# avi2924/Speech-Intent-Recognizer

Measured on AMD Instinct MI355X. Metric: utterances/sec (16 kHz, 3 s clips), inference: HIP STFT+mel+CNN/BiGRU forward + argmax, higher is better.
Workload: dtype f32

## Files before the change

speech-intent-recognizer_amd/csrc/api.hip:

```cpp
#include "sir_internal.h"
#include "model_shape.h"

#include <math.h>
#include <stdarg.h>
#include <stdio.h>
#include <string.h>
#include <algorithm>
#include <vector>

static thread_local char g_err[512] = "";

void sir_set_error(const char* fmt, ...) {
    va_list ap;
    va_start(ap, fmt);
    vsnprintf(g_err, sizeof(g_err), fmt, ap);
    va_end(ap);
}

int sir_check_hip(hipError_t e, const char* what) {
    if (e == hipSuccess) return SIR_OK;
    sir_set_error("HIP error %d (%s) at %s", (int)e, hipGetErrorString(e), what);
    return SIR_EHIP;
}

extern "C" int sir_abi_version(void) { return SIR_ABI_VERSION; }
extern "C" const char* sir_last_error(void) { return g_err; }

template <typename T>
static int upload(T** dst, const std::vector<T>& src) {
    SIR_HIP_TRY(hipMalloc((void**)dst, src.size() * sizeof(T)));
    SIR_HIP_TRY(hipMemcpy(*dst, src.data(), src.size() * sizeof(T), hipMemcpyHostToDevice));
    return SIR_OK;
}

bool sir_conv_stage_fits(int conv, bool shape_ok) {
    static const int forced = getenv("SIR_CONV_FALLBACK") ? atoi(getenv("SIR_CONV_FALLBACK")) : 0;
    return shape_ok && forced < (conv == 2 ? 1 : 2);
}

extern "C" int sir_create(const sir_feature_config* cfg, sir_handle** out) { return sir_create_ex(cfg, 0, out); }

extern "C" int sir_create_ex(const sir_feature_config* cfg, int win_length, sir_handle** out) {
    if (!cfg || !out) { sir_set_error("sir_create: NULL argument"); return SIR_EINVAL; }
    const int n_fft = cfg->n_fft, hop = cfg->hop_length;
    if (win_length == 0) win_length = n_fft;
    if ((n_fft != 256 && n_fft != 512 && n_fft != 1024) || hop < n_fft / 16 || hop > n_fft || win_length < 1 || win_length > n_fft) {
        sir_set_error("sir_create: n_fft=%d hop_length=%d win_length=%d is not built; supported: n_fft in {256, 512, 1024}, "
                      "n_fft/16 <= hop_length <= n_fft, 1 <= win_length <= n_fft", n_fft, hop, win_length);
        return SIR_EUNSUPPORTED;
    }
    if (cfg->n_mels < 1 || cfg->n_mels > SIR_MAX_MELS || cfg->sample_rate <= 0) {
        sir_set_error("sir_create: n_mels=%d sample_rate=%d out of range", cfg->n_mels, cfg->sample_rate);
        return SIR_EINVAL;
    }
    const int nfreq = n_fft / 2 + 1;
    sir_handle* h = new sir_handle();
    h->prof_mode = 0; h->prof_only = -1;
    h->weights_version = 0; h->prep_next = 0;
    for (auto& e : h->prep) { e.ws = nullptr; e.version = 0; e.key = -1; }
    h->tw512 = nullptr; h->tw1024 = nullptr; h->window = nullptr; h->melw = nullptr; h->mel_desc = nullptr;
    h->mel_taps = nullptr; h->mel_max_cover = 0;
    h->win_length = win_length;
    h->general = !(n_fft == SIR_NFFT && hop == SIR_HOP && win_length == SIR_NFFT);
    h->gen_twn = nullptr; h->gen_tw2n = nullptr;
    h->status = nullptr;
    h->cluster_done = nullptr; h->cluster_stream = nullptr; h->cluster_pending = false;
    h->cluster_seen = false; h->cluster_multi = false; h->cluster_run = 0;
    h->zero_page = nullptr; h->num_cus = 256;
    for (auto& x : h->xbufs) { x.st = nullptr; x.p = nullptr; x.kind = 0; x.cap = 0; x.bytes = 0; x.epoch = 0; x.used = 0; }
    h->xbuf_clock = 0;
    h->xbuf_evictions = 0;
    h->bwd_side = nullptr;
    for (auto& e : h->bwd_ev) e = nullptr;
    h->cfg = *cfg;
    h->cfg.window = nullptr;
    h->cfg.mel_fb = nullptr;
    if (sir_check_hip(hipGetDevice(&h->device), "hipGetDevice") != SIR_OK) { delete h; return SIR_EHIP; }

    const double PI = 3.14159265358979323846;
    std::vector<float2> tw512(512), tw1024(SIR_NFREQ);
    for (int j = 0; j < 512; ++j) tw512[j] = make_float2((float)cos(-2.0 * PI * j / 512.0), (float)sin(-2.0 * PI * j / 512.0));
    for (int k = 0; k < SIR_NFREQ; ++k) tw1024[k] = make_float2((float)cos(-2.0 * PI * k / 1024.0), (float)sin(-2.0 * PI * k / 1024.0));
    std::vector<float> window(n_fft, 0.0f);
    const int wleft = (n_fft - win_length) / 2;
    for (int n = 0; n < win_length; ++n)
        window[wleft + n] = cfg->window ? cfg->window[n] : (float)(0.5 - 0.5 * cos(2.0 * PI * n / win_length));
    std::vector<float2> gen_twn, gen_tw2n;
    if (h->general) {
        const int np = n_fft / 2;
        gen_twn.resize(np); gen_tw2n.resize(np);
        for (int k = 0; k < np; ++k) {
            gen_twn[k] = make_float2((float)cos(-2.0 * PI * k / np), (float)sin(-2.0 * PI * k / np));
            gen_tw2n[k] = make_float2((float)cos(-2.0 * PI * k / n_fft), (float)sin(-2.0 * PI * k / n_fft));
        }
    }

    const int nm = cfg->n_mels;
    std::vector<float> fb((size_t)nfreq * nm);
    if (cfg->mel_fb) {
        memcpy(fb.data(), cfg->mel_fb, fb.size() * sizeof(float));
    } else {
        const double f_lo = cfg->f_min, f_hi = cfg->f_max > 0 ? cfg->f_max : cfg->sample_rate / 2;
        const double mmin = 2595.0 * log10(1.0 + f_lo / 700.0), mmax = 2595.0 * log10(1.0 + f_hi / 700.0);
        std::vector<double> fpts(nm + 2);
        for (int i = 0; i < nm + 2; ++i) fpts[i] = 700.0 * (pow(10.0, (mmin + (mmax - mmin) * i / (nm + 1)) / 2595.0) - 1.0);
        for (int k = 0; k < nfreq; ++k) {
            const double f = (double)(cfg->sample_rate / 2) * k / (nfreq - 1);
            for (int j = 0; j < nm; ++j) {
                const double up = (f - fpts[j]) / (fpts[j + 1] - fpts[j]), down = (fpts[j + 2] - f) / (fpts[j + 2] - fpts[j + 1]);
                const double v = up < down ? up : down;
                fb[(size_t)k * nm + j] = (float)(v > 0.0 ? v : 0.0);
            }
        }
    }
    std::vector<int> start(SIR_MAX_MELS, 0), count(SIR_MAX_MELS, 0);
    for (int j = 0; j < nm; ++j) {
        int lo = -1, hi = -1;
        for (int k = 0; k < nfreq; ++k)
            if (fb[(size_t)k * nm + j] != 0.0f) { if (lo < 0) lo = k; hi = k; }
        if (lo >= 0) { start[j] = lo; count[j] = hi - lo + 1; }
    }
    std::vector<int> order(SIR_MAX_MELS);
    for (int j = 0; j < SIR_MAX_MELS; ++j) order[j] = j;
    std::stable_sort(order.begin(), order.end(), [&](int a, int b) {
        const int ca = a < nm ? count[a] : -1, cb = b < nm ? count[b] : -1;
        return ca < cb;
    });
    std::vector<float> melw;
    std::vector<int4> desc(SIR_MAX_MELS);
    for (int s = 0; s < SIR_MAX_MELS; ++s) {
        const int j = order[s];
        if (j >= nm) { desc[s] = make_int4(-1, 0, 0, 0); continue; }
        desc[s] = make_int4(j, start[j], count[j], (int)melw.size());
        for (int i = 0; i < count[j]; ++i) melw.push_back(fb[(size_t)(start[j] + i) * nm + j]);
    }
    if (melw.size() > 4096) {
        sir_set_error("sir_create: the mel filterbank has %zu taps; only banded (triangular) banks of <= 4096 taps are built", melw.size());
        delete h;
        return SIR_EUNSUPPORTED;
    }
    h->mel_nnz = (int)melw.size();
    if (h->general && sir_features_gen_lds_bytes(n_fft, h->mel_nnz) > SIR_LDS_BYTES) {
// ... 246 lines not shown
```

speech-intent-recognizer_amd/csrc/gru_quad.hip:

```cpp
#include <stdlib.h>
#include "gru_quad_kernel.h"
#include "gru_bwd_quad_kernel.h"

int sir_launch_gru_quad(sir_handle* h, hipStream_t st, bool save, const float* gi, const float* whh0, const float* whh1, const float* bhh0,
                        const float* bhh1, float* y, int B, int S, float* gates, unsigned short* yplanes, const void* wfrag0,
                        const void* wfrag1, const int* nlive, bool ragged) {
    if (ragged && (save || !nlive)) { sir_set_error("gru_quad: the ragged form is inference only and needs the step counts"); return SIR_EINVAL; }
    if (S >= 511) { sir_set_error("gru_quad: %d steps exceed the 9-bit step field of the granule tag", S); return SIR_EUNSUPPORTED; }
    if (!wfrag0 || !wfrag1) { sir_set_error("gru_quad: the prepared W_hh fragments are required (sir_prep_whh_quad / train_prep_kernel)"); return SIR_EINVAL; }
    const int clusters = ((B + GQ_NU - 1) / GQ_NU) * 2;
    const dim3 grid(4 * (unsigned)clusters);
    static const int dbg0 = getenv("SIR_GRU_DBG") ? atoi(getenv("SIR_GRU_DBG")) : 0;
    const int dbg = (dbg0 & ~(31 << 8)) | ((((dbg0 >> 8) & 31) ? ((dbg0 >> 8) & 31) : GQ_POLL_DELAY) << 8);
    typedef void (*kern_t)(const float*, const float*, const float*, const float*, const float*, float*, int, int, float*, unsigned long long*,
                           unsigned int*, int, unsigned, unsigned short*, const uint4*, const uint4*, const int*);
    const kern_t kern = save ? gru_quad_kernel<true, true> : ragged ? gru_quad_kernel<false, false, true> : gru_quad_kernel<false, false>;
    SIR_TRY(sir_lds_opt_in(h, (const void*)kern, (int)GQ_LDS_BYTES));
    SIR_TRY(sir_cluster_enter(h, st));
    unsigned epoch = 0;
    void* xbuf = nullptr;
    int rc = sir_xbuf_acquire(h, st, 1, (size_t)clusters * GQ_XBUF_PER_CLUSTER, 127u, &xbuf, &epoch);
    if (rc == SIR_OK) {
        hipLaunchKernelGGL(kern, grid, dim3(GQ_THREADS), GQ_LDS_BYTES, st, gi, whh0, whh1, bhh0, bhh1, y, B, S, gates,
                           (unsigned long long*)xbuf, h->status, dbg, epoch, yplanes, (const uint4*)wfrag0, (const uint4*)wfrag1, nlive);
        rc = sir_check_hip(hipGetLastError(), "gru_quad_kernel");
    }
    const int rc_leave = sir_cluster_leave(h, st);
    return rc != SIR_OK ? rc : rc_leave;
}

void sir_prep_whh_quad(hipStream_t st, const float* whh, void* frag) {
    hipLaunchKernelGGL(prep_whh_quad_kernel, dim3(GQ_FRAG_THREADS / 256), dim3(256), 0, st, whh, (uint4*)frag);
}

int sir_launch_gru_bwd_quad(sir_handle* h, hipStream_t st, const float* dy, const float* gates, const float* y, const float* whh0,
                            const float* whh1, float* dgi, float* dgh, float* bsum_i, float* bsum_h, int B, int S, const void* wfrag0,
                            const void* wfrag1) {
    if (S >= 65535) { sir_set_error("gru_bwd_quad: %d steps exceed the 16-bit step field of the granule tag", S); return SIR_EUNSUPPORTED; }
    if (!wfrag0 || !wfrag1) { sir_set_error("gru_bwd_quad: the prepared W_hh fragments are required (train_prep_kernel)"); return SIR_EINVAL; }
    const int clusters = ((B + GQ_NU - 1) / GQ_NU) * 2;
    const int dbg = GQ_POLL_DELAY << 8;
    SIR_TRY(sir_lds_opt_in(h, (const void*)gru_bwd_quad_kernel, (int)BQ_LDS_BYTES));
    SIR_TRY(sir_cluster_enter(h, st));
    unsigned epoch = 0;
    void* xbuf = nullptr;
    int rc = sir_xbuf_acquire(h, st, 3, (size_t)clusters * BQ_XBUF_PER_CLUSTER, 0xFFFFu, &xbuf, &epoch);
    if (rc == SIR_OK) {
        hipLaunchKernelGGL(gru_bwd_quad_kernel, dim3(4 * (unsigned)clusters), dim3(GQ_THREADS), BQ_LDS_BYTES, st, dy, gates, y, whh0, whh1, dgi, dgh,
                           bsum_i, bsum_h, B, S, (unsigned long long*)xbuf, h->status, epoch, dbg, (const uint4*)wfrag0, (const uint4*)wfrag1);
        rc = sir_check_hip(hipGetLastError(), "gru_bwd_quad_kernel");
    }
    const int rc_leave = sir_cluster_leave(h, st);
    return rc != SIR_OK ? rc : rc_leave;
}
```

speech-intent-recognizer_amd/csrc/gru_quad_kernel.h:

```cpp
#pragma once
#include "bf16x6_kernels.h"
#include "gru_frag_prep.h"

typedef unsigned int gq_u32x4 __attribute__((ext_vector_type(4)));
constexpr int GQ_NU = 16;
constexpr int GQ_UQ = 64;
constexpr int GQ_THREADS = 256;
constexpr int GQ_ROWB = 256 * 2 + 32;
constexpr int GQ_PLANEB = GQ_NU * GQ_ROWB;
constexpr int GQ_NPL = 2;
constexpr int GQ_BUFB = GQ_NPL * GQ_PLANEB;
constexpr size_t GQ_LDS_PLANES = 2 * (size_t)GQ_BUFB;
constexpr int GQ_TROW = 64 + 4;
constexpr size_t GQ_LDS_BYTES = GQ_LDS_PLANES + (size_t)GQ_NU * 3 * GQ_TROW * 4;
constexpr unsigned GQ_SPIN_LIMIT = 1u << 22;
constexpr int GQ_POLL_DELAY = 8;
constexpr size_t GQ_XBUF_PER_CLUSTER = (size_t)2 * 4 * GQ_NU * GQ_UQ * 8;

typedef float f32x4_t __attribute__((ext_vector_type(4)));

__device__ __forceinline__ void gq_mfma_aw(f32x4_t& acc, const f16x8& w, const f16x8& h) {
    asm volatile("v_mfma_f32_16x16x32_f16 %0, %1, %2, %0" : "+v"(acc) : "a"(w), "v"(h));
}
__device__ __forceinline__ void gq_mfma_wa(f32x4_t& acc, const f16x8& h, const f16x8& w) {
    asm volatile("v_mfma_f32_16x16x32_f16 %0, %1, %2, %0" : "+v"(acc) : "v"(h), "a"(w));
}
__device__ __forceinline__ void gq_mfma_enter(f32x4_t (&a)[3], f32x4_t (&b)[3]) {
    asm volatile("s_nop 3" : "+v"(a[0]), "+v"(a[1]), "+v"(a[2]), "+v"(b[0]), "+v"(b[1]), "+v"(b[2]));
}
__device__ __forceinline__ void gq_mfma_fence(f32x4_t (&a)[3], f32x4_t (&b)[3]) {
    asm volatile("s_nop 15" : "+v"(a[0]), "+v"(a[1]), "+v"(a[2]), "+v"(b[0]), "+v"(b[1]), "+v"(b[2]));
}
__device__ __forceinline__ void gq_mfma_enter(f32x4_t (&a)[4], f32x4_t (&b)[4]) {
    asm volatile("s_nop 3" : "+v"(a[0]), "+v"(a[1]), "+v"(a[2]), "+v"(a[3]), "+v"(b[0]), "+v"(b[1]), "+v"(b[2]), "+v"(b[3]));
}
__device__ __forceinline__ void gq_mfma_fence(f32x4_t (&a)[4], f32x4_t (&b)[4]) {
    asm volatile("s_nop 15" : "+v"(a[0]), "+v"(a[1]), "+v"(a[2]), "+v"(a[3]), "+v"(b[0]), "+v"(b[1]), "+v"(b[2]), "+v"(b[3]));
}

__device__ __forceinline__ float gq_sigmoid(float x) {
    return __builtin_amdgcn_rcpf(1.0f + __builtin_amdgcn_exp2f(-1.44269504088896341f * x));
}
__device__ __forceinline__ float gq_tanh(float x) {
    return 1.0f - 2.0f * __builtin_amdgcn_rcpf(1.0f + __builtin_amdgcn_exp2f(2.88539008177792681f * x));
}

static __global__ __launch_bounds__(256) void prep_whh_quad_kernel(const float* __restrict__ whh, uint4* __restrict__ frag) {
    prep_whh_quad_elem(whh, frag, blockIdx.x * 256 + threadIdx.x);
}

template <bool SAVE, bool ROLES = false, bool RAGGED = false>
__global__ __launch_bounds__(GQ_THREADS) void gru_quad_kernel(
    const float* __restrict__ gi, const float* __restrict__ whh0, const float* __restrict__ whh1,
    const float* __restrict__ bhh0, const float* __restrict__ bhh1, float* __restrict__ y, int B, int S,
    float* __restrict__ gates, unsigned long long* xbuf, unsigned int* status, int dbg, unsigned epoch, unsigned short* __restrict__ yplanes,
    const uint4* __restrict__ wfrag0, const uint4* __restrict__ wfrag1, const int* __restrict__ nlive) {
    extern __shared__ __attribute__((aligned(16))) unsigned char qlds[];
    const int nclusters = gridDim.x >> 2;
    const bool xcd_order = (nclusters & 7) == 0 && !(dbg & 32);
    const int q = xcd_order ? (blockIdx.x >> 3) & 3 : blockIdx.x & 3;
    const int cluster = xcd_order ? (blockIdx.x & 7) + 8 * (blockIdx.x >> 5) : blockIdx.x >> 2;
    const int dir = cluster & 1, grp = cluster >> 1;
    const int tid = threadIdx.x, lane = tid & 63, wv = tid >> 6;
    const int n = lane & 15, kg = lane >> 4;
    const int gutt = ROLES ? 4 * wv + (lane >> 4) : n;
    const int gul0 = ROLES ? 4 * (lane & 15) : wv * 16 + kg * 4;
    const int b = grp * GQ_NU + gutt;
    const bool bvalid = b < B;
    const int u0 = q * GQ_UQ + gul0;
    float* const tl = reinterpret_cast<float*>(qlds + GQ_LDS_PLANES);
    const float* __restrict__ bhh = dir ? bhh1 : bhh0;
    unsigned long long* xc = xbuf + (size_t)cluster * (2 * 4 * GQ_NU * GQ_UQ);

    int sr_ = S;
    if constexpr (RAGGED) {
        const int ui = grp * GQ_NU + (lane & 15);
        sr_ = ui < B ? min(S, nlive[ui]) : 0;
#pragma unroll
        for (int o = 8; o > 0; o >>= 1) sr_ = max(sr_, __shfl_xor(sr_, o));
        sr_ = max(sr_, min(S, 2));
    }
    const int SR = sr_;

    f16x8 wf[3][8][GQ_NPL];
    {
        const uint4* wsrc = (dir ? wfrag1 : wfrag0) + (size_t)((q * 4 + wv) * 3 * 8 * GQ_NPL) * 64 + lane;
#pragma unroll
        for (int g = 0; g < 3; ++g)
#pragma unroll
            for (int s = 0; s < 8; ++s)
#pragma unroll
                for (int p = 0; p < GQ_NPL; ++p)
                    asm volatile("global_load_dwordx4 %0, %1, off" : "=a"(wf[g][s][p]) : "v"(wsrc + ((g * 8 + s) * GQ_NPL + p) * 64));
        asm volatile("s_waitcnt vmcnt(0)" ::: "memory");
    }
    float4 bh[3];
#pragma unroll
    for (int g = 0; g < 3; ++g) bh[g] = *reinterpret_cast<const float4*>(bhh + g * 256 + u0);
    for (int i = tid; i < (int)(GQ_LDS_BYTES / 16); i += GQ_THREADS) reinterpret_cast<uint4*>(qlds)[i] = make_uint4(0, 0, 0, 0);
    float4 hprev = make_float4(0.f, 0.f, 0.f, 0.f);
    __syncthreads();

    float4 gin[3];
    const int nlb = (!SAVE && nlive && bvalid) ? nlive[b] : (RAGGED ? 0 : S);
    auto load_gi = [&](int t, float4 (&dst)[3]) {
#pragma unroll
        for (int g = 0; g < 3; ++g) dst[g] = make_float4(0.f, 0.f, 0.f, 0.f);
        if (RAGGED ? (bvalid && t < nlb) : bvalid) {
            const float* gp = gi + ((size_t)(RAGGED || t < nlb ? b : B) * S + t) * 1536 + dir * 768 + u0;
#pragma unroll
            for (int g = 0; g < 3; ++g) dst[g] = *reinterpret_cast<const float4*>(gp + g * 256);
        }
    };
    load_gi(dir ? SR - 1 : 0, gin);
    const int frag_off = n * GQ_ROWB + kg * 16;
    const int xoff = wv * 256 + lane * 2;
    bool timed_out = false;

    for (int step = 0; step < SR; ++step) {
        const int t = dir ? (SR - 1 - step) : step;
        float4 gcur[3] = {gin[0], gin[1], gin[2]};
        const unsigned char* hb = qlds + (step & 1) * GQ_BUFB;
        unsigned char* hnb = qlds + ((step + 1) & 1) * GQ_BUFB;

        f32x4_t acc[3], accx[3];
#pragma unroll
        for (int g = 0; g < 3; ++g) { acc[g] = (f32x4_t){0.f, 0.f, 0.f, 0.f}; accx[g] = (f32x4_t){0.f, 0.f, 0.f, 0.f}; }
        f16x8 hf[8][GQ_NPL];
        if (!(dbg & 2)) {
#pragma unroll
        for (int s = 0; s < 8; ++s)
#pragma unroll
            for (int p = 0; p < GQ_NPL; ++p)
                hf[s][p] = __builtin_bit_cast(f16x8, *reinterpret_cast<const uint4*>(hb + p * GQ_PLANEB + frag_off + s * 64));
        __builtin_amdgcn_sched_barrier(0);
        gq_mfma_enter(acc, accx);
#pragma unroll
        for (int s = 0; s < 8; ++s) {
#pragma unroll
            for (int g = 0; g < 3; ++g) gq_mfma_aw(accx[g], wf[g][s][1], hf[s][0]);
#pragma unroll
            for (int g = 0; g < 3; ++g) gq_mfma_aw(accx[g], wf[g][s][0], hf[s][1]);
#pragma unroll
            for (int g = 0; g < 3; ++g) gq_mfma_aw(acc[g], wf[g][s][0], hf[s][0]);
        }
        gq_mfma_fence(acc, accx);
#pragma unroll
        for (int g = 0; g < 3; ++g)
#pragma unroll
            for (int j = 0; j < 4; ++j) acc[g][j] = fmaf(accx[g][j], H3_LO_INV, acc[g][j]);
        }
        if constexpr (ROLES) {
#pragma unroll
            for (int g = 0; g < 3; ++g)
                *reinterpret_cast<float4*>(tl + (n * 3 + g) * GQ_TROW + wv * 16 + kg * 4) = make_float4(acc[g][0], acc[g][1], acc[g][2], acc[g][3]);
            __syncthreads();
#pragma unroll
            for (int g = 0; g < 3; ++g) {
                const float4 v = *reinterpret_cast<const float4*>(tl + (gutt * 3 + g) * GQ_TROW + gul0);
                acc[g][0] = v.x; acc[g][1] = v.y; acc[g][2] = v.z; acc[g][3] = v.w;
            }
        }

        float hn4[4], r4[4], z4[4], n4[4], hh4[4];
        const float gr[4] = {gcur[0].x, gcur[0].y, gcur[0].z, gcur[0].w}, gz[4] = {gcur[1].x, gcur[1].y, gcur[1].z, gcur[1].w};
        const float gn[4] = {gcur[2].x, gcur[2].y, gcur[2].z, gcur[2].w};
        const float br[4] = {bh[0].x, bh[0].y, bh[0].z, bh[0].w}, bz[4] = {bh[1].x, bh[1].y, bh[1].z, bh[1].w};
        const float bn[4] = {bh[2].x, bh[2].y, bh[2].z, bh[2].w};
        const float hp[4] = {hprev.x, hprev.y, hprev.z, hprev.w};
#pragma unroll
        for (int j = 0; j < 4; ++j) {
            const float hr = acc[0][j] + br[j], hz = acc[1][j] + bz[j];
            hh4[j] = acc[2][j] + bn[j];
            r4[j] = gq_sigmoid(gr[j] + hr);
            z4[j] = gq_sigmoid(gz[j] + hz);
            n4[j] = gq_tanh(gn[j] + r4[j] * hh4[j]);
            hn4[j] = (1.0f - z4[j]) * n4[j] + z4[j] * hp[j];
            if (RAGGED) hn4[j] = t < nlb ? hn4[j] : hp[j];
        }
        hprev = make_float4(hn4[0], hn4[1], hn4[2], hn4[3]);

        uint2 ph, pl;
        split2h_quad(hprev, ph, pl);
        {
// ... 92 lines not shown
```

speech-intent-recognizer_amd/csrc/model_infer.hip:

```cpp
#include "f16x3_kernels.h"
#include "conv_fwd.h"
#include "gru_frag_prep.h"

namespace {

enum WsBuf {
    WS_A1 = 0,
    WS_A2,
    WS_X0,
    WS_GI,
    WS_Y0,
    WS_Y1,
    WS_CTX,
    WS_PAD,
    WS_XZ,
    WS_BN,
    WS_WHT,
    WS_XS,
    WS_WS,
    WS_WCB,
    WS_GXB,
    WS_GFL,
    WS_COUNT
};

struct Dims : SirDims {
    int tw2, tw3, k2max, k3max;
};

bool make_dims(int batch, int t_frames, Dims* d) {
    if (!sir_make_dims(batch, t_frames, d)) return false;
    d->tw2 = (d->wp1 + 1) / 2; d->tw3 = (d->wp2 + 1) / 2; d->k2max = (d->tw2 + 3) / 4; d->k3max = (d->tw3 + 3) / 4;
    return true;
}

struct PadTabs { size_t e0, d1, d3, tab2, tab3, rows, count; };
PadTabs pad_tabs(const Dims& d) {
    PadTabs t;
    const size_t n = (size_t)d.B + 1;
    t.e0 = 0; t.d1 = d.B; t.d3 = t.d1 + n; t.rows = t.d3 + n + 1 + n * d.k2max + 1 + n * d.k3max;
    t.tab2 = t.rows + 1 + n * d.S; t.tab2 += t.tab2 & 1;
    t.tab3 = t.tab2 + 2 + 2 * n * d.k2max;
    t.count = t.tab3 + 2 + 2 * n * d.k3max;
    return t;
}

void ws_sizes(const Dims& d, size_t* bytes) {
    const size_t B = d.B + 1;
    bytes[WS_A1] = B * 32 * d.wp1 * 32 * 4;
    bytes[WS_A2] = B * 16 * d.wp2 * 64 * 4;
    bytes[WS_X0] = B * d.S * 1024 * 4;
    bytes[WS_GI] = B * d.S * 1536 * 4;
    bytes[WS_Y0] = (size_t)d.B * d.S * 512 * 4;
    bytes[WS_Y1] = (size_t)d.B * d.S * 512 * 4;
    bytes[WS_CTX] = (size_t)d.B * 512 * 4;
    bytes[WS_PAD] = pad_tabs(d).count * 4;
    bytes[WS_XZ] = (size_t)64 * d.T * 4;
    bytes[WS_BN] = (size_t)2 * 224 * 4;
    bytes[WS_WHT] = 4 * GRU_FRAG_BYTES;
    bytes[WS_XS] = B * d.S * 1024 * 2 * 2;
    bytes[WS_WS] = ((size_t)2 * 2 * 768 * 1024 + (size_t)2 * 2 * 768 * 512) * 2;
    bytes[WS_WCB] = ((size_t)3 * 32 * 16 * 64 + (size_t)3 * 64 * 16 * 128 + (size_t)3 * 64 * 9 * 128) * 2;
    bytes[WS_GXB] = 0;
    bytes[WS_GFL] = 0;
}

size_t ws_layout(const Dims& d, size_t* off) {
    size_t bytes[WS_COUNT], pos = 0;
    ws_sizes(d, bytes);
    for (int i = 0; i < WS_COUNT; ++i) {
        off[i] = pos;
        pos += sir_align_up(bytes[i], 256);
    }
    return pos;
}

static __global__ __launch_bounds__(256) void pad_extent_kernel(const float* __restrict__ x, int T, int* __restrict__ e0) {
    const unsigned* xb = reinterpret_cast<const unsigned*>(x) + (size_t)blockIdx.x * 64 * T;
    int last = -1;
    for (int c = threadIdx.x; c < T; c += 256) {
        unsigned acc = 0;
#pragma unroll 32
        for (int r = 0; r < 64; ++r) acc |= xb[(size_t)r * T + c];
        if (acc) last = c;
    }
#pragma unroll
    for (int o = 32; o > 0; o >>= 1) last = max(last, __shfl_xor(last, o));
    __shared__ int wl[4];
    if ((threadIdx.x & 63) == 0) wl[threadIdx.x >> 6] = last;
    __syncthreads();
    if (threadIdx.x == 0) e0[blockIdx.x] = max(max(wl[0], wl[1]), max(wl[2], wl[3])) + 1;
}

__device__ __forceinline__ int pk_cap(int r) { const int l = r & 3; return l == 1 ? 2 : l == 2 ? 1 : 0; }
__device__ __forceinline__ int pk_take(int c, int g, int cn) { return g <= c ? min(pk_cap(c - g), cn) : 0; }
constexpr int PK_ID = 0 | 1 << 2 | 2 << 4;
__device__ __forceinline__ int pk_fn(int c, int cn) { return pk_take(c, 0, cn) | pk_take(c, 1, cn) << 2 | pk_take(c, 2, cn) << 4; }
__device__ __forceinline__ int pk_then(int f, int g) {
    int r = 0;
#pragma unroll
    for (int x = 0; x < 3; ++x) r |= ((g >> (2 * ((f >> (2 * x)) & 3))) & 3) << (2 * x);
    return r;
}
__device__ __forceinline__ void pk_emit(int* __restrict__ tab, int o, int base, int g, int r, int gB, int nB) {
    const int k = (r + 3) >> 2;
    for (int t = 0; t < k; ++t) {
        reinterpret_cast<int2*>(tab)[1 + o + t] = make_int2((base + g + 4 * t) << 2 | (min(4, r - 4 * t) - 1),
                                                            t == k - 1 && nB > 0 ? gB << 2 | (2 - nB) << 1 | (nB - 1) : -1);
    }
}

template <bool PACK, typename Need>
__device__ __forceinline__ void pad_tables_emit(const Dims& d, int nu, Need need, int* __restrict__ d1o, int* __restrict__ d3o,
                                                int* __restrict__ tab2, int* __restrict__ tab3, int* __restrict__ prow) {
    const int tid = threadIdx.x;
    const int per = (nu + 1023) / 1024, u0 = min(nu, tid * per), u1 = min(nu, u0 + per);
    const int nr = PACK ? nu - 1 : nu;
    __shared__ int wt[3][16];
    auto scan = [&](auto op, int id, int& a, int& b, int& c, int& ta, int& tb, int& tc) {
        const int ln = tid & 63, wv = tid >> 6;
#pragma unroll
        for (int o = 1; o < 64; o <<= 1) {
            const int xa = __shfl_up(a, o), xb = __shfl_up(b, o), xc = __shfl_up(c, o);
            if (ln >= o) { a = op(xa, a); b = op(xb, b); c = op(xc, c); }
        }
        __syncthreads();
        if (ln == 63) { wt[0][wv] = a; wt[1][wv] = b; wt[2][wv] = c; }
        __syncthreads();
        int pa = id, pb = id, pc = id;
        ta = id; tb = id; tc = id;
        for (int w = 0; w < 16; ++w) {
            const int va = wt[0][w], vb = wt[1][w], vc = wt[2][w];
            if (w < wv) { pa = op(pa, va); pb = op(pb, vb); pc = op(pc, vc); }
            ta = op(ta, va); tb = op(tb, vb); tc = op(tc, vc);
        }
        const int xa = __shfl_up(a, 1), xb = __shfl_up(b, 1), xc = __shfl_up(c, 1);
        a = ln ? op(pa, xa) : pa; b = ln ? op(pb, xb) : pb; c = ln ? op(pc, xc) : pc;
    };
    auto add = [](int a, int b) { return a + b; };
    int c1, c2, c3, n1, n2, n3;
    int q2_0 = 0, q3_0 = 0, orw0 = 0, cap2, cap3, nrow;
    for (int u = u0; u < u1; ++u) { need(u, c1, c2, c3); orw0 += c3; if (PACK && u < nr) { q2_0 += pk_cap(c2); q3_0 += pk_cap(c3); } }
    scan(add, 0, q2_0, q3_0, orw0, cap2, cap3, nrow);
    int t2 = 0, t3 = 0, gt2 = 0, gt3 = 0;
    if (PACK) { need(nr, c1, t2, t3); gt2 = min(t2, cap2); gt3 = min(t3, cap3); }
    int g2 = 0, g3 = 0;
    if (PACK) {
// ... 56 lines not shown
                                                                    int* __restrict__ d3o, int* __restrict__ tab2, int* __restrict__ tab3,
                                                                    int* __restrict__ prow, unsigned int* __restrict__ status) {
    bool bad = false;
    for (int u = threadIdx.x; u < d.B; u += 1024) {
        const int f0 = frames[u], f = f0 >= 8 && f0 <= d.T ? f0 : 0;
        fw[u] = f;
        bad |= f == 0;
    }
    if (bad) __hip_atomic_fetch_or(status, 64u, __ATOMIC_RELAXED, __HIP_MEMORY_SCOPE_AGENT);
    __syncthreads();
    auto need = [&](int u, int& c1, int& c2, int& c3) {
        const int f = fw[u];
        c1 = f >> 1; c2 = f >> 2; c3 = f >> 3;
    };
    pad_tables_emit<false>(d, d.B, need, d1o, d3o, tab2, tab3, prow);
}

static __global__ __launch_bounds__(256) void ragged_mask_kernel(float* __restrict__ a, const int* __restrict__ fw, int sh, int H, int W, int C) {
    const int b = blockIdx.y, r = blockIdx.x, w0 = min(W, fw[b] >> sh);
    float4* row = reinterpret_cast<float4*>(a + (((size_t)b * H + r) * W + w0) * C);
    const int n4 = (W - w0) * (C / 4);
    for (int i = threadIdx.x; i < n4; i += 256) row[i] = make_float4(0.0f, 0.0f, 0.0f, 0.0f);
}

}

extern "C" size_t sir_model_workspace_bytes(const sir_handle* h, int batch, int t_frames, int train) {
    (void)h;
    if (train) return sir_train_workspace_bytes_impl(batch, t_frames);
    Dims d;
    if (!make_dims(batch, t_frames, &d)) return 0;
    size_t off[WS_COUNT];
    return ws_layout(d, off);
}

extern "C" int sir_model_workspace_offsets(const sir_handle* h, int batch, int t_frames, int train, size_t* offsets,
                                           int n) {
    (void)h; (void)train;
    Dims d;
    if (!make_dims(batch, t_frames, &d) || !offsets) { sir_set_error("sir_model_workspace_offsets: bad shape"); return SIR_EINVAL; }
    size_t off[WS_COUNT];
    ws_layout(d, off);
    for (int i = 0; i < n && i < WS_COUNT; ++i) offsets[i] = off[i];
    return WS_COUNT;
}

static int model_infer_impl(const char* who, sir_handle* h, const sir_model_weights* w, const float* feats, const int32_t* frames, int batch,
                            int t_frames, float* logits, int64_t* argmax, void* workspace, size_t workspace_bytes, void* stream_) {
    if (!h || !w || !feats || !logits || !workspace) { sir_set_error("%s: NULL argument", who); return SIR_EINVAL; }
    Dims d;
    if (!make_dims(batch, t_frames, &d)) {
        sir_set_error("%s: unsupported shape batch=%d t_frames=%d (need t_frames >= 8)", who, batch, t_frames);
        return SIR_EINVAL;
    }
    if (h->cfg.n_mels != 64) { sir_set_error("%s: the model is wired for 64 mels (models.py:23)", who); return SIR_EUNSUPPORTED; }
    if (w->num_classes < 1 || w->num_classes > 64) { sir_set_error("%s: num_classes=%d", who, w->num_classes); return SIR_EINVAL; }
    size_t off[WS_COUNT];
    const size_t need = ws_layout(d, off);
    if (workspace_bytes < need) { sir_set_error("%s: workspace %zu < %zu", who, workspace_bytes, need); return SIR_ENOMEM; }
    if (((uintptr_t)workspace & 255) != 0) { sir_set_error("%s: workspace must be 256-byte aligned", who); return SIR_EINVAL; }
    const bool ragged = frames != nullptr;
    hipStream_t st = (hipStream_t)stream_;
    char* ws = (char*)workspace;
    float* a1 = (float*)(ws + off[WS_A1]);
    float* a2 = (float*)(ws + off[WS_A2]);
    float* x0 = (float*)(ws + off[WS_X0]);
    float* gi = (float*)(ws + off[WS_GI]);
    float* y0 = (float*)(ws + off[WS_Y0]);
    float* y1 = (float*)(ws + off[WS_Y1]);
    float* ctx = (float*)(ws + off[WS_CTX]);
    float* bns = (float*)(ws + off[WS_BN]);
    float* bnt = bns + 224;
    float* wht = (float*)(ws + off[WS_WHT]);
    unsigned short* xs = (unsigned short*)(ws + off[WS_XS]);
    unsigned short* wsl0 = (unsigned short*)(ws + off[WS_WS]);
    unsigned short* wsl1 = wsl0 + (size_t)2 * 2 * 768 * 1024;
    unsigned short* wcb2 = (unsigned short*)(ws + off[WS_WCB]);
    unsigned short* wcb3 = wcb2 + (size_t)3 * 32 * 16 * 64;
    unsigned short* wcb3d = wcb3 + (size_t)3 * 64 * 16 * 128;
    const int B = d.B, S = d.S;
    const PadTabs pt = pad_tabs(d);
    int* const ptab = (int*)(ws + off[WS_PAD]);
    float* const xz = (float*)(ws + off[WS_XZ]);

    const SirConvPlan cp = sir_conv_plan(&d, true);
    const bool w2 = cp.fwd_wino;
    const int BT = w2 ? B + 1 : B;

    const long long prep_key = ((long long)B << 32) | (unsigned)d.T;
    sir_handle::PrepEntry* pe = nullptr;
    for (auto& e : h->prep)
        if (e.ws == workspace) pe = &e;
    const bool reuse_prep = pe && h->weights_version != 0 && pe->version == h->weights_version && pe->key == prep_key;
    if (!reuse_prep) {
        SirProfScope prof(h, SIR_K_PREP, st);
        const int bn_c[3] = {32, 64, 128}, bn_o[3] = {0, 32, 96};
        for (int i = 0; i < 3; ++i)
            hipLaunchKernelGGL(prep_bn_kernel, dim3(1), dim3(128), 0, st, w->bn_w[i], w->bn_b[i], w->bn_mean[i], w->bn_var[i],
                               bns + bn_o[i], bnt + bn_o[i], bn_c[i]);
        for (int i = 0; i < 4; ++i) sir_prep_whh_quad(st, w->gru_w_hh[i], (unsigned char*)wht + (size_t)i * GRU_FRAG_BYTES);
        if (w2) hipLaunchKernelGGL(prep_conv_w_wino_f16x3_kernel, dim3((32 * 16 * 64 + 255) / 256), dim3(256), 0, st, w->conv_w[1], wcb2, 32, 64, h->status);
        else hipLaunchKernelGGL(prep_conv_w_wino_bf16x3_kernel, dim3((32 * 16 * 64 + 255) / 256), dim3(256), 0, st, w->conv_w[1], wcb2, 32, 64);
        if (w2) hipLaunchKernelGGL(prep_conv_w_wino_f16x3_kernel, dim3((64 * 16 * 128 + 255) / 256), dim3(256), 0, st, w->conv_w[2], wcb3, 64, 128, h->status);
        else hipLaunchKernelGGL(prep_conv_w_wino_bf16x3_kernel, dim3((64 * 16 * 128 + 255) / 256), dim3(256), 0, st, w->conv_w[2], wcb3, 64, 128);
        hipLaunchKernelGGL(prep_conv_w_bf16x3_kernel, dim3((64 * 9 * 128 + 255) / 256), dim3(256), 0, st, w->conv_w[2], wcb3d, 64, 128);
        for (int dir = 0; dir < 2; ++dir) {
            hipLaunchKernelGGL(split2h_kernel, dim3(384), dim3(256), 0, st, w->gru_w_ih[dir], 1024, wsl0 + (size_t)dir * 2 * 768 * 1024, (size_t)768, 1024);
            hipLaunchKernelGGL(split2h_kernel, dim3(192), dim3(256), 0, st, w->gru_w_ih[2 + dir], 512, wsl1 + (size_t)dir * 2 * 768 * 512, (size_t)768, 512);
        }
        if (!pe) { pe = &h->prep[h->prep_next]; h->prep_next = (h->prep_next + 1) % 4; }
        pe->ws = workspace; pe->version = h->weights_version; pe->key = prep_key;
    }
    SIR_KCHECK();

    {
        SirProfScope prof(h, SIR_K_CONV1, st);
        if (ragged) {
            hipLaunchKernelGGL(ragged_tables_kernel, dim3(1), dim3(1024), 0, st, (const int*)frames, d, ptab + pt.e0, ptab + pt.d1, ptab + pt.d3,
                               ptab + pt.tab2, ptab + pt.tab3, ptab + pt.rows, h->status);
            hipLaunchKernelGGL(conv1_mfma_bn_relu_pool_ragged_kernel, conv1_grid(B, d.wp1), dim3(256), 0, st, feats,
                               w->conv_w[0], bns, bnt, a1, 64, d.T, 32, d.wp1, (const int*)(ptab + pt.d1), (const int*)(ptab + pt.e0));
            if (!w2) hipLaunchKernelGGL(ragged_mask_kernel, dim3(32, B), dim3(256), 0, st, a1, (const int*)(ptab + pt.e0), 1, 32, d.wp1, 32);
        } else {
        if (w2) {
            hipLaunchKernelGGL(pad_extent_kernel, dim3(B), dim3(256), 0, st, feats, d.T, ptab + pt.e0);
            hipLaunchKernelGGL(pad_tables_kernel, dim3(1), dim3(1024), 0, st, (const int*)(ptab + pt.e0), d, ptab + pt.d1, ptab + pt.d3,
                               ptab + pt.tab2, ptab + pt.tab3, ptab + pt.rows, xz);
        }
        hipLaunchKernelGGL(conv1_mfma_bn_relu_pool_kernel, conv1_grid(BT, d.wp1), dim3(256), 0, st, feats,
                           w->conv_w[0], bns, bnt, a1, 64, d.T, 32, d.wp1, (const float*)xz, B, w2 ? (const int*)(ptab + pt.d1) : (const int*)nullptr);
        }
    }
    {
        SirProfScope prof(h, SIR_K_CONV2, st);
        if (ragged) {
            SIR_TRY((conv_fwd<32, 64, 0, true>(h, st, w2, cp.geo2, B, a1, wcb2, nullptr, bns + 32, bnt + 32, a2, nullptr, ptab + pt.tab2, (B + 1) * d.k2max,
                                               ptab + pt.e0, 1)));
            if (!w2) hipLaunchKernelGGL(ragged_mask_kernel, dim3(16, B), dim3(256), 0, st, a2, (const int*)(ptab + pt.e0), 2, 16, d.wp2, 64);
        } else
        SIR_TRY((conv_fwd<32, 64, 0>(h, st, w2, cp.geo2, BT, a1, wcb2, nullptr, bns + 32, bnt + 32, a2, nullptr, ptab + pt.tab2, (B + 1) * d.k2max)));
    }
    {
        SirProfScope prof(h, SIR_K_CONV3, st);
        if (ragged)
            SIR_TRY((conv_fwd<64, 128, 1, true>(h, st, w2, cp.geo3, B, a2, wcb3, wcb3d, bns + 96, bnt + 96, x0, (float2*)xs, ptab + pt.tab3, (B + 1) * d.k3max,
                                                ptab + pt.e0, 2)));
        else
        SIR_TRY((conv_fwd<64, 128, 1>(h, st, w2, cp.geo3, BT, a2, wcb3, wcb3d, bns + 96, bnt + 96, x0, (float2*)xs, ptab + pt.tab3, (B + 1) * d.k3max)));
    }
    SIR_KCHECK();

    const int M = B * S;
    {
        SirProfScope prof(h, SIR_K_GEMM_IH0, st);
        if (w2 || ragged)
            SIR_TRY(launch_gemm_nt_f16x3_gather(h, st, (const unsigned short*)xs, (const unsigned short*)wsl0,
                                                    (const unsigned short*)(wsl0 + (size_t)2 * 768 * 1024), w->gru_b_ih[0], w->gru_b_ih[1], gi, 1536,
                                                    (const int*)(ptab + pt.rows), BT * S, 768, 1024));
        else
            SIR_TRY(launch_gemm_nt_f16x3(h, st, (const unsigned short*)xs, (const unsigned short*)wsl0,
                                             (const unsigned short*)(wsl0 + (size_t)2 * 768 * 1024), w->gru_b_ih[0], w->gru_b_ih[1], gi, 1536, M, 768, 1024));
    }
    {
        SirProfScope prof(h, SIR_K_GRU0, st);
        SIR_TRY(sir_launch_gru_quad(h, st, false, gi, w->gru_w_hh[0], w->gru_w_hh[1], w->gru_b_hh[0], w->gru_b_hh[1], y0, B, S, nullptr,
                                    xs, wht, (unsigned char*)wht + GRU_FRAG_BYTES, w2 || ragged ? (const int*)(ptab + pt.d3) : (const int*)nullptr, ragged));
    }
    {
        SirProfScope prof(h, SIR_K_GEMM_IH1, st);
        if (ragged)
            SIR_TRY(launch_gemm_nt_f16x3_gather(h, st, (const unsigned short*)xs, (const unsigned short*)wsl1,
                                                    (const unsigned short*)(wsl1 + (size_t)2 * 768 * 512), w->gru_b_ih[2], w->gru_b_ih[3], gi, 1536,
                                                    (const int*)(ptab + pt.rows), M, 768, 512));
        else
        SIR_TRY(launch_gemm_nt_f16x3(h, st, (const unsigned short*)xs, (const unsigned short*)wsl1,
                                         (const unsigned short*)(wsl1 + (size_t)2 * 768 * 512), w->gru_b_ih[2], w->gru_b_ih[3], gi, 1536, M, 768, 512));
    }
    {
        SirProfScope prof(h, SIR_K_GRU1, st);
        SIR_TRY(sir_launch_gru_quad(h, st, false, gi, w->gru_w_hh[2], w->gru_w_hh[3], w->gru_b_hh[2], w->gru_b_hh[3], y1, B, S, nullptr,
                                    nullptr, (unsigned char*)wht + 2 * GRU_FRAG_BYTES, (unsigned char*)wht + 3 * GRU_FRAG_BYTES,
                                    ragged ? (const int*)(ptab + pt.d3) : (const int*)nullptr, ragged));
    }
    SIR_KCHECK();

    {
        SirProfScope prof(h, SIR_K_ATTN, st);
        if (ragged)
            hipLaunchKernelGGL(attention_pool_ragged_kernel, dim3(B), dim3(256), 0, st, y1, w->attn_w, w->attn_b, ctx, S, w->fc_w, w->fc_b,
                               w->num_classes, logits, (long long*)argmax, (const int*)(ptab + pt.d3));
        else
        hipLaunchKernelGGL(attention_pool_kernel, dim3(B), dim3(256), 0, st, y1, w->attn_w, w->attn_b, ctx, S, w->fc_w, w->fc_b,
                           w->num_classes, logits, (long long*)argmax);
    }
    SIR_KCHECK();
    return SIR_OK;
}

extern "C" int sir_model_infer(sir_handle* h, const sir_model_weights* w, const float* feats, int batch, int t_frames,
                               float* logits, int64_t* argmax, void* workspace, size_t workspace_bytes, void* stream_) {
    return model_infer_impl("sir_model_infer", h, w, feats, nullptr, batch, t_frames, logits, argmax, workspace, workspace_bytes, stream_);
}

extern "C" int sir_model_infer_ragged(sir_handle* h, const sir_model_weights* w, const float* feats, const int32_t* frames, int batch,
                                      int t_frames, float* logits, int64_t* argmax, void* workspace, size_t workspace_bytes,
                                      void* stream_) {
    if (!frames) { sir_set_error("sir_model_infer_ragged: NULL frames"); return SIR_EINVAL; }
    return model_infer_impl("sir_model_infer_ragged", h, w, feats, frames, batch, t_frames, logits, argmax, workspace, workspace_bytes, stream_);
}
```

speech-intent-recognizer_amd/csrc/sir_internal.h:

```cpp
#pragma once
#include <hip/hip_runtime.h>
#include <stdint.h>
#include <stddef.h>
#include <vector>
#include "sir_hip.h"

void sir_set_error(const char* fmt, ...);

#define SIR_WAVE 64
#define SIR_NFFT 1024
#define SIR_HOP 512
#define SIR_NFREQ 513
#define SIR_MAX_MELS 64

enum SirKernelId {
    SIR_K_FEAT_FRAMES = 0, SIR_K_FEAT_NORM, SIR_K_PREP, SIR_K_CONV1, SIR_K_CONV2, SIR_K_CONV3,
    SIR_K_GEMM_IH0, SIR_K_GRU0, SIR_K_GEMM_IH1, SIR_K_GRU1, SIR_K_ATTN, SIR_K_FC,
    SIR_K_T_PREP, SIR_K_T_CONV1, SIR_K_T_CONV2, SIR_K_T_BN2, SIR_K_T_CONV3, SIR_K_T_BN3, SIR_K_T_GEMM_IH0, SIR_K_T_GRU0,
    SIR_K_T_DROPOUT, SIR_K_T_GEMM_IH1, SIR_K_T_GRU1, SIR_K_T_HEAD, SIR_K_CE,
    SIR_K_B_HEAD, SIR_K_B_GRU1, SIR_K_B_DW1, SIR_K_B_DX1, SIR_K_B_GRU0, SIR_K_B_DW0, SIR_K_B_DX0,
    SIR_K_B_BN3, SIR_K_B_WGRAD3, SIR_K_B_DGRAD3, SIR_K_B_BN2, SIR_K_B_WGRAD2, SIR_K_B_DGRAD2, SIR_K_B_CONV1, SIR_K_ADAM,
    SIR_K_MIX, SIR_K_GRAD_SUMSQ, SIR_K_GRAD_CLIP, SIR_K_ADAM_CLIPPED,
    SIR_K_ADAM_EX, SIR_K_ADAM_EX_CLIPPED,
    SIR_K_VAD_ENERGY, SIR_K_VAD_SEGMENT, SIR_K_VAD_GATHER,
    SIR_K_COUNT,
    SIR_K_B_CONV1_DGRAD = SIR_K_COUNT,
    SIR_K_COUNT_ALL
};
static_assert(SIR_K_COUNT_ALL - SIR_K_COUNT == SIR_PROFILE_EXTRA_IDS, "include/sir_hip.h: SIR_PROFILE_EXTRA_IDS");

struct SirProfRec { int id; hipEvent_t e0, e1; };
static inline size_t sir_align_up(size_t x, size_t a) { return (x + a - 1) / a * a; }

struct sir_resample_table {
    int orig_freq, new_freq;
    int orig, nw, width, L;
    float* taps;
    int* first;
};

struct sir_handle {
    int prof_mode;
    int prof_only;
    std::vector<SirProfRec> prof_pending;
    std::vector<hipEvent_t> prof_free;
    unsigned long long weights_version;
    struct PrepEntry { const void* ws; unsigned long long version; long long key; };
    PrepEntry prep[4];
    int prep_next;
    sir_feature_config cfg;
    int device;
    float2* tw512;
    float2* tw1024;
    float* window;
    float* melw;
    int4* mel_desc;
    int mel_nnz;
    int win_length;
    bool general;
    float2* gen_twn;
    float2* gen_tw2n;
    void* mel_taps;
    int mel_max_cover;
    std::vector<sir_resample_table> resample_tables;
    unsigned int* status;
    hipEvent_t cluster_done;
    hipStream_t cluster_stream;
    bool cluster_pending, cluster_seen, cluster_multi;
    int cluster_run;
    std::vector<const void*> lds_opted;
    float* zero_page;
    int num_cus;
    struct XbufEntry { hipStream_t st; int kind; void* p; size_t cap, bytes; unsigned epoch; unsigned long long used; };
    XbufEntry xbufs[16];
    unsigned long long xbuf_clock;
    unsigned long long xbuf_evictions;
    hipStream_t bwd_side;
    hipEvent_t bwd_ev[6];
};

static inline int sir_xbuf_acquire(sir_handle* h, hipStream_t st, int kind, size_t bytes, unsigned mask, void** xbuf, unsigned* epoch) {
    sir_handle::XbufEntry* e = nullptr;
    for (auto& x : h->xbufs)
        if (x.p && x.st == st && x.kind == kind) e = &x;
    if (!e) {
        e = &h->xbufs[0];
        for (auto& x : h->xbufs) {
            if (!x.p) { e = &x; break; }
            if (x.used < e->used) e = &x;
        }
        if (e->p) {
            ++h->xbuf_evictions;
            if (hipFree(e->p) != hipSuccess) { sir_set_error("exchange buffer: hipFree of an evicted buffer failed"); return SIR_EHIP; }
            e->p = nullptr;
        }
        e->st = st; e->kind = kind; e->cap = 0; e->bytes = 0; e->epoch = 0;
    }
    if (bytes > e->cap) {
        if (e->p && hipFree(e->p) != hipSuccess) { sir_set_error("exchange buffer: hipFree before growing failed"); return SIR_EHIP; }
        e->p = nullptr; e->cap = 0; e->bytes = 0;
        const size_t cap = sir_align_up(bytes, (size_t)1 << 20);
        if (hipMalloc(&e->p, cap) != hipSuccess) { e->p = nullptr; sir_set_error("exchange buffer: hipMalloc of %zu bytes failed", cap); return SIR_EHIP; }
        e->cap = cap;
    }
    if (bytes > e->bytes && hipMemsetAsync(e->p, 0, bytes, st) != hipSuccess) { sir_set_error("exchange buffer: hipMemsetAsync failed"); return SIR_EHIP; }
    e->bytes = bytes;
    e->epoch = (e->epoch + 1) & mask;
    e->used = ++h->xbuf_clock;
    *epoch = e->epoch;
    *xbuf = e->p;
    return SIR_OK;
}

static inline int sir_cluster_enter(sir_handle* h, hipStream_t st) {
    if (!h->cluster_multi) {
        if (h->cluster_seen && h->cluster_stream != st) {
            if (hipDeviceSynchronize() != hipSuccess) return SIR_EHIP;
            h->cluster_multi = true;
            h->cluster_pending = false;
            h->cluster_run = 0;
        }
        return SIR_OK;
    }
    if (h->cluster_pending && h->cluster_stream != st)
        if (hipStreamWaitEvent(st, h->cluster_done, 0) != hipSuccess) return SIR_EHIP;
    return SIR_OK;
}
static inline int sir_cluster_leave(sir_handle* h, hipStream_t st) {
    if (h->cluster_multi) {
        if (hipEventRecord(h->cluster_done, st) != hipSuccess) return SIR_EHIP;
        h->cluster_pending = true;
        h->cluster_run = (h->cluster_stream == st) ? h->cluster_run + 1 : 0;
        if (h->cluster_run >= 64) { h->cluster_multi = false; h->cluster_pending = false; }
    }
    h->cluster_stream = st;
    h->cluster_seen = true;
    return SIR_OK;
}

int sir_check_hip(hipError_t e, const char* what);

#define SIR_HIP_TRY(expr)                                   \
    do {                                                    \
        int _rc = sir_check_hip((expr), #expr);             \
        if (_rc != SIR_OK) return _rc;                      \
    } while (0)
#define SIR_KCHECK() SIR_HIP_TRY(hipGetLastError())
#define SIR_TRY(expr)                                       \
    do {                                                    \
        int _rc = (expr);                                   \
        if (_rc != SIR_OK) return _rc;                      \
    } while (0)

static inline int sir_lds_opt_in(sir_handle* h, const void* kernel, int bytes) {
    for (const void* k : h->lds_opted)
        if (k == kernel) return SIR_OK;
    SIR_HIP_TRY(hipFuncSetAttribute(kernel, hipFuncAttributeMaxDynamicSharedMemorySize, bytes));
    h->lds_opted.push_back(kernel);
    return SIR_OK;
}

struct SirProfScope {
    sir_handle* h; int id; hipStream_t st; hipEvent_t e0, e1; bool on;
    SirProfScope(sir_handle* h_, int id_, hipStream_t st_) : h(h_), id(id_), st(st_), e0(nullptr), e1(nullptr) {
        on = h->prof_mode == 1 || (h->prof_mode == 2 && h->prof_only == id);
        if (!on) return;
        hipEvent_t ev[2];
        for (int i = 0; i < 2; ++i) {
            if (!h->prof_free.empty()) { ev[i] = h->prof_free.back(); h->prof_free.pop_back(); }
            else if (hipEventCreate(&ev[i]) != hipSuccess) { on = false; return; }
        }
        e0 = ev[0]; e1 = ev[1];
        (void)hipEventRecord(e0, st);
    }
    ~SirProfScope() {
        if (!on) return;
        (void)hipEventRecord(e1, st);
        h->prof_pending.push_back(SirProfRec{id, e0, e1});
    }
};

size_t sir_train_workspace_bytes_impl(int batch, int t_frames);

size_t sir_features_gen_lds_bytes(int n_fft, int mel_nnz);
#define SIR_LDS_BYTES (160 * 1024)
int sir_features_launch(sir_handle* h, const void* wave, int wave_dtype, int64_t wave_stride,
                        const int32_t* lengths, int batch, int max_len, float* out, int t_pad,
                        float* db_out, void* workspace, size_t workspace_bytes, const sir_augment* aug,
                        hipStream_t stream);
int sir_features_bwd_launch(sir_handle* h, const void* wave, int wave_dtype, int64_t wave_stride, const int32_t* lengths,
                            int batch, int max_len, const float* db, const float* dout, int t_pad, const sir_augment* aug,
                            float* dwave, int64_t dwave_stride, hipStream_t stream);

int sir_launch_gru_quad(sir_handle* h, hipStream_t st, bool save, const float* gi, const float* whh0, const float* whh1, const float* bhh0,
                        const float* bhh1, float* y, int B, int S, float* gates,
                        unsigned short* yplanes = nullptr, const void* wfrag0 = nullptr, const void* wfrag1 = nullptr,
                        const int* nlive = nullptr, bool ragged = false);
void sir_prep_whh_quad(hipStream_t st, const float* whh, void* frag);
int sir_launch_gru_bwd_quad(sir_handle* h, hipStream_t st, const float* dy, const float* gates, const float* y, const float* whh0,
                            const float* whh1, float* dgi, float* dgh, float* bsum_i, float* bsum_h, int B, int S,
                            const void* wfrag0 = nullptr, const void* wfrag1 = nullptr);
```

Measured before the change: 763,200.

## Reuse a cached padding trajectory to skip padded steps in the backward GRU

Adds a TPL variant of the padded-inference GRU kernel. It computes, once per prepared-weights entry, the backward-direction hidden-state trajectory over pure padding frames and stores it in a new workspace slot. On later calls the backward direction copies the cached outputs and bf16 planes for the padded tail. It then seeds its LDS state and h_prev from the trajectory at each utterance's live length and runs only the live steps. This removes serial recurrent steps over padding, at the cost of extra global copies and the assumption that padded frames give identical GRU inputs.

Result: no change. 766,100 (median of 2 runs) (+0.4%).

```diff
diff --git a/speech-intent-recognizer_amd/csrc/api.hip b/speech-intent-recognizer_amd/csrc/api.hip
--- a/speech-intent-recognizer_amd/csrc/api.hip
+++ b/speech-intent-recognizer_amd/csrc/api.hip
@@ -57,7 +57,7 @@
     sir_handle* h = new sir_handle();
     h->prof_mode = 0; h->prof_only = -1;
     h->weights_version = 0; h->prep_next = 0;
-    for (auto& e : h->prep) { e.ws = nullptr; e.version = 0; e.key = -1; }
+    for (auto& e : h->prep) { e.ws = nullptr; e.version = 0; e.key = -1; e.traj = false; }
     h->tw512 = nullptr; h->tw1024 = nullptr; h->window = nullptr; h->melw = nullptr; h->mel_desc = nullptr;
     h->mel_taps = nullptr; h->mel_max_cover = 0;
     h->win_length = win_length;
diff --git a/speech-intent-recognizer_amd/csrc/gru_quad.hip b/speech-intent-recognizer_amd/csrc/gru_quad.hip
--- a/speech-intent-recognizer_amd/csrc/gru_quad.hip
+++ b/speech-intent-recognizer_amd/csrc/gru_quad.hip
@@ -4,7 +4,9 @@
 
 int sir_launch_gru_quad(sir_handle* h, hipStream_t st, bool save, const float* gi, const float* whh0, const float* whh1, const float* bhh0,
                         const float* bhh1, float* y, int B, int S, float* gates, unsigned short* yplanes, const void* wfrag0,
-                        const void* wfrag1, const int* nlive, bool ragged) {
+                        const void* wfrag1, const int* nlive, bool ragged, const float* trajy, const unsigned short* trajpl) {
+    const bool tpl = trajy != nullptr;
+    if (tpl != (trajpl != nullptr) || (tpl && (save || ragged || !nlive))) { sir_set_error("gru_quad: the template trajectory belongs to the padded inference form with step counts"); return SIR_EINVAL; }
     if (ragged && (save || !nlive)) { sir_set_error("gru_quad: the ragged form is inference only and needs the step counts"); return SIR_EINVAL; }
     if (S >= 511) { sir_set_error("gru_quad: %d steps exceed the 9-bit step field of the granule tag", S); return SIR_EUNSUPPORTED; }
     if (!wfrag0 || !wfrag1) { sir_set_error("gru_quad: the prepared W_hh fragments are required (sir_prep_whh_quad / train_prep_kernel)"); return SIR_EINVAL; }
@@ -13,8 +15,9 @@
     static const int dbg0 = getenv("SIR_GRU_DBG") ? atoi(getenv("SIR_GRU_DBG")) : 0;
     const int dbg = (dbg0 & ~(31 << 8)) | ((((dbg0 >> 8) & 31) ? ((dbg0 >> 8) & 31) : GQ_POLL_DELAY) << 8);
     typedef void (*kern_t)(const float*, const float*, const float*, const float*, const float*, float*, int, int, float*, unsigned long long*,
-                           unsigned int*, int, unsigned, unsigned short*, const uint4*, const uint4*, const int*);
-    const kern_t kern = save ? gru_quad_kernel<true, true> : ragged ? gru_quad_kernel<false, false, true> : gru_quad_kernel<false, false>;
+                           unsigned int*, int, unsigned, unsigned short*, const uint4*, const uint4*, const int*, const float*, const unsigned short*);
+    const kern_t kern = save ? gru_quad_kernel<true, true> : ragged ? gru_quad_kernel<false, false, true>
+                      : tpl ? gru_quad_kernel<false, false, false, true> : gru_quad_kernel<false, false>;
     SIR_TRY(sir_lds_opt_in(h, (const void*)kern, (int)GQ_LDS_BYTES));
     SIR_TRY(sir_cluster_enter(h, st));
     unsigned epoch = 0;
@@ -22,7 +25,7 @@
     int rc = sir_xbuf_acquire(h, st, 1, (size_t)clusters * GQ_XBUF_PER_CLUSTER, 127u, &xbuf, &epoch);
     if (rc == SIR_OK) {
         hipLaunchKernelGGL(kern, grid, dim3(GQ_THREADS), GQ_LDS_BYTES, st, gi, whh0, whh1, bhh0, bhh1, y, B, S, gates,
-                           (unsigned long long*)xbuf, h->status, dbg, epoch, yplanes, (const uint4*)wfrag0, (const uint4*)wfrag1, nlive);
+                           (unsigned long long*)xbuf, h->status, dbg, epoch, yplanes, (const uint4*)wfrag0, (const uint4*)wfrag1, nlive, trajy, trajpl);
         rc = sir_check_hip(hipGetLastError(), "gru_quad_kernel");
     }
     const int rc_leave = sir_cluster_leave(h, st);
diff --git a/speech-intent-recognizer_amd/csrc/gru_quad_kernel.h b/speech-intent-recognizer_amd/csrc/gru_quad_kernel.h
--- a/speech-intent-recognizer_amd/csrc/gru_quad_kernel.h
+++ b/speech-intent-recognizer_amd/csrc/gru_quad_kernel.h
@@ -49,12 +49,13 @@
     prep_whh_quad_elem(whh, frag, blockIdx.x * 256 + threadIdx.x);
 }
 
-template <bool SAVE, bool ROLES = false, bool RAGGED = false>
+template <bool SAVE, bool ROLES = false, bool RAGGED = false, bool TPL = false>
 __global__ __launch_bounds__(GQ_THREADS) void gru_quad_kernel(
     const float* __restrict__ gi, const float* __restrict__ whh0, const float* __restrict__ whh1,
     const float* __restrict__ bhh0, const float* __restrict__ bhh1, float* __restrict__ y, int B, int S,
     float* __restrict__ gates, unsigned long long* xbuf, unsigned int* status, int dbg, unsigned epoch, unsigned short* __restrict__ yplanes,
-    const uint4* __restrict__ wfrag0, const uint4* __restrict__ wfrag1, const int* __restrict__ nlive) {
+    const uint4* __restrict__ wfrag0, const uint4* __restrict__ wfrag1, const int* __restrict__ nlive,
+    const float* __restrict__ trajy, const unsigned short* __restrict__ trajpl) {
     extern __shared__ __attribute__((aligned(16))) unsigned char qlds[];
     const int nclusters = gridDim.x >> 2;
     const bool xcd_order = (nclusters & 7) == 0 && !(dbg & 32);
@@ -72,8 +73,9 @@
     const float* __restrict__ bhh = dir ? bhh1 : bhh0;
     unsigned long long* xc = xbuf + (size_t)cluster * (2 * 4 * GQ_NU * GQ_UQ);
 
+    static_assert(!TPL || (!SAVE && !ROLES && !RAGGED), "TPL is a variant of the padded inference form");
     int sr_ = S;
-    if constexpr (RAGGED) {
+    if (RAGGED || (TPL && dir)) {
         const int ui = grp * GQ_NU + (lane & 15);
         sr_ = ui < B ? min(S, nlive[ui]) : 0;
 #pragma unroll
@@ -100,6 +102,32 @@
     for (int i = tid; i < (int)(GQ_LDS_BYTES / 16); i += GQ_THREADS) reinterpret_cast<uint4*>(qlds)[i] = make_uint4(0, 0, 0, 0);
     float4 hprev = make_float4(0.f, 0.f, 0.f, 0.f);
     __syncthreads();
+    if constexpr (TPL) {
+        if (dir && SR < S) {
+            const int ub = grp * GQ_NU + (tid >> 4);
+            if (ub < B) {
+                const size_t plane = (size_t)B * S * 512, tplane = (size_t)S * 512;
+                const int uo = 256 + q * GQ_UQ + (tid & 15) * 4;
+#pragma unroll 4
+                for (int t = SR; t < S; ++t) {
+                    const size_t so = (size_t)t * 512 + uo, yo = ((size_t)ub * S + t) * 512 + uo;
+                    *reinterpret_cast<float4*>(y + yo) = *reinterpret_cast<const float4*>(trajy + so);
+                    if (yplanes) {
+                        *reinterpret_cast<uint2*>(yplanes + yo) = *reinterpret_cast<const uint2*>(trajpl + so);
+                        *reinterpret_cast<uint2*>(yplanes + plane + yo) = *reinterpret_cast<const uint2*>(trajpl + tplane + so);
+                    }
+                }
+            }
+            const size_t trow = (size_t)SR * 512 + 256;
+            for (int i = tid; i < GQ_NPL * GQ_NU * 32; i += GQ_THREADS) {
+                const int c = i & 31, r = (i >> 5) & 15, p = i >> 9;
+                *reinterpret_cast<uint4*>(qlds + p * GQ_PLANEB + r * GQ_ROWB + c * 16) =
+                    *reinterpret_cast<const uint4*>(trajpl + (size_t)p * S * 512 + trow + c * 8);
+            }
+            hprev = *reinterpret_cast<const float4*>(trajy + trow + u0);
+            __syncthreads();
+        }
+    }
 
     float4 gin[3];
     const int nlb = (!SAVE && nlive && bvalid) ? nlive[b] : (RAGGED ? 0 : S);
diff --git a/speech-intent-recognizer_amd/csrc/model_infer.hip b/speech-intent-recognizer_amd/csrc/model_infer.hip
--- a/speech-intent-recognizer_amd/csrc/model_infer.hip
+++ b/speech-intent-recognizer_amd/csrc/model_infer.hip
@@ -21,6 +21,7 @@
     WS_WCB,
     WS_GXB,
     WS_GFL,
+    WS_TRAJ,
     WS_COUNT
 };
 
@@ -63,6 +64,7 @@
     bytes[WS_WCB] = ((size_t)3 * 32 * 16 * 64 + (size_t)3 * 64 * 16 * 128 + (size_t)3 * 64 * 9 * 128) * 2;
     bytes[WS_GXB] = 0;
     bytes[WS_GFL] = 0;
+    bytes[WS_TRAJ] = (size_t)d.S * 512 * (4 + 2 * 2);
 }
 
 size_t ws_layout(const Dims& d, size_t* off) {
@@ -285,6 +287,8 @@
     const PadTabs pt = pad_tabs(d);
     int* const ptab = (int*)(ws + off[WS_PAD]);
     float* const xz = (float*)(ws + off[WS_XZ]);
+    float* const trajy = (float*)(ws + off[WS_TRAJ]);
+    unsigned short* const trajpl = (unsigned short*)(trajy + (size_t)d.S * 512);
 
     const SirConvPlan cp = sir_conv_plan(&d, true);
     const bool w2 = cp.fwd_wino;
@@ -312,7 +316,7 @@
             hipLaunchKernelGGL(split2h_kernel, dim3(192), dim3(256), 0, st, w->gru_w_ih[2 + dir], 512, wsl1 + (size_t)dir * 2 * 768 * 512, (size_t)768, 512);
         }
         if (!pe) { pe = &h->prep[h->prep_next]; h->prep_next = (h->prep_next + 1) % 4; }
-        pe->ws = workspace; pe->version = h->weights_version; pe->key = prep_key;
+        pe->ws = workspace; pe->version = h->weights_version; pe->key = prep_key; pe->traj = false;
     }
     SIR_KCHECK();
 
@@ -364,10 +368,18 @@
             SIR_TRY(launch_gemm_nt_f16x3(h, st, (const unsigned short*)xs, (const unsigned short*)wsl0,
                                              (const unsigned short*)(wsl0 + (size_t)2 * 768 * 1024), w->gru_b_ih[0], w->gru_b_ih[1], gi, 1536, M, 768, 1024));
     }
+    const bool tpl = w2 && !ragged;
+    if (tpl && !pe->traj) {
+        SirProfScope prof(h, SIR_K_PREP, st);
+        SIR_TRY(sir_launch_gru_quad(h, st, false, gi + (size_t)B * S * 1536, w->gru_w_hh[0], w->gru_w_hh[1], w->gru_b_hh[0], w->gru_b_hh[1], trajy, 1, S,
+                                    nullptr, trajpl, wht, (unsigned char*)wht + GRU_FRAG_BYTES));
+        pe->traj = true;
+    }
     {
         SirProfScope prof(h, SIR_K_GRU0, st);
         SIR_TRY(sir_launch_gru_quad(h, st, false, gi, w->gru_w_hh[0], w->gru_w_hh[1], w->gru_b_hh[0], w->gru_b_hh[1], y0, B, S, nullptr,
-                                    xs, wht, (unsigned char*)wht + GRU_FRAG_BYTES, w2 || ragged ? (const int*)(ptab + pt.d3) : (const int*)nullptr, ragged));
+                                    xs, wht, (unsigned char*)wht + GRU_FRAG_BYTES, w2 || ragged ? (const int*)(ptab + pt.d3) : (const int*)nullptr, ragged,
+                                    tpl ? trajy : nullptr, tpl ? trajpl : nullptr));
     }
     {
         SirProfScope prof(h, SIR_K_GEMM_IH1, st);
diff --git a/speech-intent-recognizer_amd/csrc/sir_internal.h b/speech-intent-recognizer_amd/csrc/sir_internal.h
--- a/speech-intent-recognizer_amd/csrc/sir_internal.h
+++ b/speech-intent-recognizer_amd/csrc/sir_internal.h
@@ -45,7 +45,7 @@
     std::vector<SirProfRec> prof_pending;
     std::vector<hipEvent_t> prof_free;
     unsigned long long weights_version;
-    struct PrepEntry { const void* ws; unsigned long long version; long long key; };
+    struct PrepEntry { const void* ws; unsigned long long version; long long key; bool traj; };
     PrepEntry prep[4];
     int prep_next;
     sir_feature_config cfg;
@@ -195,7 +195,8 @@
 int sir_launch_gru_quad(sir_handle* h, hipStream_t st, bool save, const float* gi, const float* whh0, const float* whh1, const float* bhh0,
                         const float* bhh1, float* y, int B, int S, float* gates,
                         unsigned short* yplanes = nullptr, const void* wfrag0 = nullptr, const void* wfrag1 = nullptr,
-                        const int* nlive = nullptr, bool ragged = false);
+                        const int* nlive = nullptr, bool ragged = false, const float* trajy = nullptr,
+                        const unsigned short* trajpl = nullptr);
 void sir_prep_whh_quad(hipStream_t st, const float* whh, void* frag);
 int sir_launch_gru_bwd_quad(sir_handle* h, hipStream_t st, const float* dy, const float* gates, const float* y, const float* whh0,
                             const float* whh1, float* dgi, float* dgh, float* bsum_i, float* bsum_h, int B, int S,
```
